# tobwei/APTAI

Measured on AMD Instinct MI355X. Metric: utterances/sec (10 s @ 16 kHz) train-step, higher is better.
Workload: dtype bf16

## Files before the change

### aptai_amd/csrc/gemm.hip

```cpp
#include <stdlib.h>

#include <mutex>
#include <set>

#include "common.h"
#include "gemm_common.h"

using namespace aptai_gemm;

namespace {

#ifdef APTAI_STAMPS
__device__ unsigned long long g_stamps[4096 * 8];
#define APTAI_STAMP(slot)                                                                          \
    do {                                                                                           \
        if (threadIdx.x == 0 && blockIdx.x < 4096 && blockIdx.y == 0 && blockIdx.z == 0)           \
            g_stamps[blockIdx.x * 8 + (slot)] = wall_clock64();                                    \
    } while (0)
extern "C" int aptai_debug_read_stamps(void* host_out) {
    return hipMemcpyFromSymbol(host_out, HIP_SYMBOL(g_stamps), sizeof(g_stamps)) == hipSuccess ? 0 : 1;
}
#else
#define APTAI_STAMP(slot) do {} while (0)
#endif

void epi_trace(const GemmArgs& g, int tile) {
    static const bool on = getenv("APTAI_EPI_TRACE") != nullptr;
    if (!on) return;
    static std::mutex mu;
    static std::set<int> seen;
    const int w = g.flags | (g.out_pre ? EPX_PRE : 0) | (g.colscale_n > 0 ? EPX_CS : 0);
    std::lock_guard<std::mutex> lk(mu);
    if (!seen.insert(w).second) return;
    bool listed = false;
#define APTAI_EPI_CASE(W) listed = listed || (w == (W));
    APTAI_EPI_WORDS(APTAI_EPI_CASE)
#undef APTAI_EPI_CASE
    fprintf(stderr, "[aptai epi] flag word 0x%x (tile %d, %d x %d x %d): %s\n", w, tile, g.M, g.N, g.K, listed ? "compiled" : "RUN-TIME form");
}

template <bool A_KM, bool B_KM, bool OUT_F32, int BM_T = 128>
__device__ __forceinline__ void gemm_tile_body(GemmArgs g, const int bid, const int batch, const int split) {
    extern __shared__ __attribute__((aligned(16))) char smem[];
    APTAI_STAMP(0);
    const int tid = threadIdx.x;
    const int lane = tid & 63;
    const int wave = __builtin_amdgcn_readfirstlane(tid >> 6);
    const int wm = wave >> 1, wn = wave & 1;

    int tile_m, tile_n;
    raster2d(bid, g.tiles_m, g.tiles_n, g.raster_gm, tile_m, tile_n);
    constexpr int NI = BM_T / 32;
    constexpr int WM = BM_T / 2;
    constexpr int NA_IT = BM_T / 32;
    constexpr int A_BYTES_T = BM_T * BK * 2;
    constexpr int STAGE_T = A_BYTES_T + BN * BK * 2;
    constexpr int NPASS = BM_T / 16;
    static_assert(BM_T == 128 || (BM_T == 64 && !A_KM), "64-row tiles are built for K-contiguous A only");
    constexpr bool RING5 = A_KM && B_KM && BM_T == 128 && APTAI_GEMM_RING5;
    const int m0 = tile_m * BM_T, n0 = tile_n * BN;

    if (batch >= 0) {
        const int bo = batch / g.nb_inner, bi = batch % g.nb_inner;
        g.A += bo * g.sA[0] + bi * g.sA[1];
        g.B += bo * g.sB[0] + bi * g.sB[1];
        const long co = bo * g.sC[0] + bi * g.sC[1];
        g.C = (OUT_F32 && !(g.flags & APTAI_EPI_SPLIT_OUT)) ? (void*)((float*)g.C + co) : (void*)((bf16_t*)g.C + co);
        if (g.out_pre) g.out_pre += co;
        if (g.bias) g.bias += bo * g.sBias[0] + bi * g.sBias[1];
        if (g.residual) g.residual += bo * g.sR[0] + bi * g.sR[1];
        if (g.aux) g.aux += bo * g.sAux[0] + bi * g.sAux[1];
    }
    const int total_kt = g.K / BK;
    const int kt_begin = split * g.ktiles_per_split;
    int kt_end = kt_begin + g.ktiles_per_split;
    kt_end = kt_end < total_kt ? kt_end : total_kt;
    const int nk = kt_end - kt_begin;

    f32x4 acc[NI][4];
#pragma unroll
    for (int i = 0; i < NI; ++i)
#pragma unroll
// ... 40 lines not shown
            }
#pragma unroll
            for (int it = 0; it < 2; ++it) {
                __builtin_amdgcn_global_load_lds(GLB_PTR(hb[it]), LDS_PTR(dst + HALF_T / 2 + it * (NTHREADS * 16)), 16, 0, 0);
                hb[it] += hstepB;
            }
        };
        uint32_t frag_off[16];
        {
            const int gq = lane >> 4, li = lane & 15, qq = li >> 2, pp = li & 3;
            const int k_lo = gq * 8 + qq, k_hi = k_lo + 4;
            const int sub = (pp & 1) << 3;
#pragma unroll
            for (int f = 0; f < 8; ++f) {
                const int is_b = f >> 2, idx = f & 3;
                const int row_base = is_b ? wn * 64 + idx * 16 : wm * WM + idx * 16;
                const int ch = (row_base >> 3) + (pp >> 1);
                frag_off[2 * f] = (uint32_t)(is_b * (HALF_T / 2) + k_lo * 256 + ((ch ^ km_swz(k_lo)) << 4) + sub);
                frag_off[2 * f + 1] = (uint32_t)(is_b * (HALF_T / 2) + k_hi * 256 + ((ch ^ km_swz(k_hi)) << 4) + sub);
            }
        }
        const uint32_t ring_base = (uint32_t)(uintptr_t)(__attribute__((address_space(3))) const char*)smem;
        const int nh = 2 * nk;
        if (nh > 0) { stage_half(0); stage_half(1); }
        if (nh > 2) stage_half(2);
        int s0 = 0;
        for (int kt = 0; kt < nk; ++kt) {
            if (kt + 1 < nk) asm volatile("s_waitcnt vmcnt(4) lgkmcnt(0)" ::: "memory");
            else asm volatile("s_waitcnt vmcnt(0) lgkmcnt(0)" ::: "memory");
            __builtin_amdgcn_s_barrier();
            asm volatile("" ::: "memory");
            const int s1 = s0 + 1 >= 5 ? s0 - 4 : s0 + 1, s2 = s0 + 2 >= 5 ? s0 - 3 : s0 + 2, s3 = s0 + 3 >= 5 ? s0 - 2 : s0 + 3,
                      s4 = s0 + 4 >= 5 ? s0 - 1 : s0 + 4;
            if (2 * kt + 3 < nh) stage_half(s3);
            if (2 * kt + 4 < nh) stage_half(s4);
            if (wave_active) {
                short4v fr[2][16];
#pragma unroll
                for (int hh = 0; hh < 2; ++hh) {
                    const uint32_t base = ring_base + (uint32_t)((hh ? s1 : s0) * HALF_T);
#pragma unroll
                    for (int f = 0; f < 16; ++f)
                        asm volatile("ds_read_b64_tr_b16 %0, %1" : "=v"(fr[hh][f]) : "v"(base + frag_off[f]));
                }
#define APTAI_TIE8(h, o) "+v"(fr[h][o]), "+v"(fr[h][o + 1]), "+v"(fr[h][o + 2]), "+v"(fr[h][o + 3]), "+v"(fr[h][o + 4]), \
                         "+v"(fr[h][o + 5]), "+v"(fr[h][o + 6]), "+v"(fr[h][o + 7])
#pragma unroll
                for (int hh = 0; hh < 2; ++hh) {
                    if (hh == 0) asm volatile("s_waitcnt lgkmcnt(15)" : APTAI_TIE8(0, 0), APTAI_TIE8(0, 8));
                    else asm volatile("s_waitcnt lgkmcnt(0)" : APTAI_TIE8(1, 0), APTAI_TIE8(1, 8));
                    bf16x8 af[NI], bfr[4];
#pragma unroll
                    for (int i = 0; i < NI; ++i) {
                        const short4v lo4 = fr[hh][2 * i], hi4 = fr[hh][2 * i + 1];
                        af[i] = __builtin_bit_cast(bf16x8, (short8v){lo4[0], lo4[1], lo4[2], lo4[3], hi4[0], hi4[1], hi4[2], hi4[3]});
                    }
#pragma unroll
                    for (int j = 0; j < 4; ++j) {
                        const short4v lo4 = fr[hh][8 + 2 * j], hi4 = fr[hh][8 + 2 * j + 1];
                        bfr[j] = __builtin_bit_cast(bf16x8, (short8v){lo4[0], lo4[1], lo4[2], lo4[3], hi4[0], hi4[1], hi4[2], hi4[3]});
                    }
#pragma unroll
                    for (int i = 0; i < NI; ++i)
#pragma unroll
                        for (int j = 0; j < 4; ++j)
                            acc[i][j] = __builtin_amdgcn_mfma_f32_16x16x32_bf16(bfr[j], af[i], acc[i][j], 0, 0, 0);
                }
#undef APTAI_TIE8
            }
            s0 = s2;
        }
        asm volatile("s_waitcnt vmcnt(0) lgkmcnt(0)" ::: "memory");
        __syncthreads();
    } else {
    if (nk > 0) stage(smem);
    for (int kt = 0; kt < nk; ++kt) {
        asm volatile("s_waitcnt vmcnt(0)" ::: "memory");
        __syncthreads();
        const int cur = kt & 1;
        if (kt + 1 < nk) stage(smem + (cur ^ 1) * STAGE_T);
        const char* sa = smem + cur * STAGE_T;
        const char* sb = sa + A_BYTES_T;
        if (wave_active) {
            if constexpr (!A_KM && !B_KM && APTAI_GEMM_HOIST) {
                bf16x8 af[2][NI], bfr[2][4];
#pragma unroll
                for (int ks = 0; ks < 2; ++ks) {
#pragma unroll
                    for (int j = 0; j < 4; ++j) bfr[ks][j] = read_frag<B_KM>(sb, wn * 64 + j * 16, ks, lane);
#pragma unroll
                    for (int i = 0; i < NI; ++i) af[ks][i] = read_frag<A_KM>(sa, wm * WM + i * 16, ks, lane);
                }
                __builtin_amdgcn_sched_barrier(0);
#pragma unroll
// ... 196 lines not shown
        }
        if (late) for (int i = 0; i < g.exp_sleep; ++i) __builtin_amdgcn_s_sleep(31);
    }
#endif
    gemm_tile_body<A_KM, B_KM, OUT_F32>(g, xcd_remap(blockIdx.x, g.tiles_m * g.tiles_n), gridDim.y > 1 ? (int)blockIdx.y : -1,
                                        blockIdx.z);
}

constexpr int SMEM_M64_BYTES = 2 * (64 + BN) * BK * 2;
template <bool B_KM, bool OUT_F32>
__global__ __launch_bounds__(NTHREADS, 3) void gemm_kernel_m64(GemmArgs g) {
    gemm_tile_body<false, B_KM, OUT_F32, 64>(g, xcd_remap(blockIdx.x, g.tiles_m * g.tiles_n), gridDim.y > 1 ? (int)blockIdx.y : -1,
                                             blockIdx.z);
}

constexpr int MAX_GROUP = 8;
struct GroupArgs {
    GemmArgs p[MAX_GROUP];
    int tile_end[MAX_GROUP];
    int n, total;
};

template <bool A_KM, bool B_KM, bool OUT_F32>
__global__ __launch_bounds__(NTHREADS, 3) void gemm_grouped_kernel(GroupArgs ga) {
    const int bid = xcd_remap(blockIdx.x, ga.total);
    int pi = 0;
#pragma unroll
    for (int i = 1; i < MAX_GROUP; ++i)
        if (i < ga.n && bid >= ga.tile_end[i - 1]) pi = i;
    const int first = pi ? ga.tile_end[pi - 1] : 0;
    gemm_tile_body<A_KM, B_KM, OUT_F32>(ga.p[pi], bid - first, -1, 0);
}

__global__ void splitk_reduce_kernel(const float* __restrict__ slabs, float* __restrict__ out, long n4, long slab_stride4,
                                     int nsplit, int accumulate) {
    const long stride = (long)gridDim.x * blockDim.x;
    for (long i = (long)blockIdx.x * blockDim.x + threadIdx.x; i < n4; i += stride) {
        f32x4 s = accumulate ? ((const f32x4*)out)[i] : (f32x4){0.f, 0.f, 0.f, 0.f};
        for (int k = 0; k < nsplit; ++k) s += ((const f32x4*)slabs)[(long)k * slab_stride4 + i];
        ((f32x4*)out)[i] = s;
    }
}

template <bool B_KM, bool OUT_F32>
int launch_gemm_m64(GemmArgs g, int nbatch, int nsplit, hipStream_t stream) {
    auto kern = gemm_kernel_m64<B_KM, OUT_F32>;
    g.tiles_m = (int)ceil_div(g.M, 64);
    dim3 grid(g.tiles_m * g.tiles_n, nbatch, nsplit);
    APTAI_LAUNCH(kern, grid, dim3(NTHREADS), SMEM_M64_BYTES, stream, g);
    APTAI_CHECK_LAUNCH("gemm_kernel_m64");
    return APTAI_OK;
}

template <bool A_KM, bool B_KM, bool OUT_F32>
// ... 890 lines not shown
                      "aptai_gemm_bf16: EPI_SPLIT_OUT needs out_f32, tile 128 / 192 / 256, 3 or 6 pieces and ldc >= pieces * N (bf16 elements)");
    APTAI_REQUIRE(d->colscale_n >= 0 && d->colscale_n % 8 == 0 && d->colscale_n <= d->N && (d->colscale_n == 0 || !d->out_f32),
                  "aptai_gemm_bf16: colscale_n must be a multiple of 8 within N, bf16 output only");
    memset(&g, 0, sizeof(g));
    g.A = (const bf16_t*)d->A; g.lda = d->lda;
    g.B = (const bf16_t*)d->B; g.ldb = d->ldb;
    g.C = d->C; g.ldc = d->ldc;
    g.M = (int)d->M; g.N = (int)d->N; g.K = (int)d->K;
    g.bias = d->bias;
    g.residual = (const bf16_t*)d->residual; g.ldr = d->ldr;
    g.out_pre = (bf16_t*)d->out_pre;
    g.aux = (const bf16_t*)d->aux; g.ldaux = d->ldaux;
    g.flags = d->flags;
    g.seed0 = (uint32_t)d->seed; g.seed1 = (uint32_t)(d->seed >> 32);
    g.salt = aptai_seed_salt(stream);
    g.thr16 = drop_thr16(d->dropout_p);
    g.dscale = drop_scale(g.thr16);
    if (g.thr16 == 0) g.flags &= ~APTAI_EPI_DROPOUT;
    g.alpha = d->alpha;
    g.colscale_n = d->colscale_n; g.colscale = d->colscale;
    g.split_pieces = d->split_out_pieces;
    g.split_bcol = (d->flags & APTAI_EPI_SPLIT_OUT) ? d->split_out_bcol : 0;
    g.hash_ld = d->N; g.hash_n0 = 0;
    g.tiles_m = (int)ceil_div(d->M, BM);
    g.tiles_n = (int)ceil_div(d->N, BN);
    {
        static int raster = -2;
        if (raster == -2) {
            const char* e = getenv("APTAI_GEMM_RASTER");
            raster = e ? atoi(e) : -1;
        }
        g.raster_gm = raster;
    }
    const int total_kt = g.K / BK;
    nsplit = d->split_k > 0 ? d->split_k : 1;
    if (nsplit > total_kt) nsplit = total_kt;
    g.ktiles_per_split = (int)ceil_div(total_kt, nsplit);
    nsplit = (int)ceil_div(total_kt, g.ktiles_per_split);

    nbatch = 1;
    g.nb_inner = 1;
    if (d->batch_outer > 1 || d->batch_inner > 1) {
        const int bo = d->batch_outer > 0 ? d->batch_outer : 1, bi = d->batch_inner > 0 ? d->batch_inner : 1;
        nbatch = bo * bi;
        g.nb_inner = bi;
        for (int l = 0; l < 2; ++l) {
// ... 33 lines not shown
                a.N = n1; a.tile = 256;
                b.N = rem; b.tile = 128;
                b.B = (const char*)d->B + (d->b_kmajor ? n1 * 2 : n1 * d->ldb * 2);
                b.C = (char*)d->C + n1 * 2;
                if (d->out_pre) b.out_pre = (char*)d->out_pre + n1 * 2;
                if (d->bias) b.bias = d->bias + n1;
                if (d->residual) b.residual = (const char*)d->residual + n1 * 2;
                if (d->aux) b.aux = (const char*)d->aux + n1 * 2;
                const int rc = gemm_bf16_one(&a, stream_, d->N, 0);
                if (rc != APTAI_OK) return rc;
                return gemm_bf16_one(&b, stream_, d->N, (int)n1);
            }
        }
    }
    return gemm_bf16_one(d, stream_, d ? d->N : 0, 0);
}

static int gemm_bf16_one(const aptai_gemm_desc* d, void* stream_, long hash_ld, int hash_n0) {
    hipStream_t stream = (hipStream_t)stream_;
    GemmArgs g;
    int nbatch = 1, nsplit = 1;
    const int brc = build_args(d, g, nbatch, nsplit, stream_);
    if (brc != APTAI_OK) return brc;
    g.hash_ld = hash_ld; g.hash_n0 = hash_n0;
    const bool f32 = d->out_f32 != 0;
    float* final_out = (float*)d->C;
    int tile = d->tile;
    if (tile == 0) {
        static int env_tile = -1;
        if (env_tile < 0) {
            const char* e = getenv("APTAI_GEMM_TILE");
            env_tile = e ? atoi(e) : 0;
        }
        tile = env_tile;
    }
    if (tile == 0) {
        const long t256 = ceil_div(d->M, T2_BM) * ceil_div(d->N, T2_BN) * nbatch * nsplit;
        const long t128 = ceil_div(d->M, BM) * ceil_div(d->N, BN) * nbatch * nsplit;
        const double e256 = (double)t256 / (double)(ceil_div(t256, 256) * 256);
        const double e128 = (double)t128 / (double)(ceil_div(t128, 512) * 512);
        static double f256 = -1.0;
        if (f256 < 0) {
            const char* e = getenv("APTAI_GEMM_F256");
            f256 = e ? atof(e) : 1.25;
        }
        tile = (d->M >= 256 && d->N >= 256 && f256 * e256 > e128) ? 256 : 128;
// ... 54 lines not shown
        else if (d->a_kmajor && d->b_kmajor) rc = f32 ? launch_gemm256<true, true, true>(g, nbatch, nsplit, stream) : launch_gemm256<true, true, false>(g, nbatch, nsplit, stream);
        else APTAI_FAIL(APTAI_ERR_INVALID, "aptai_gemm_bf16: A K-major with B K-contiguous is not built");
    } else
    if (!d->a_kmajor && !d->b_kmajor) rc = f32 ? launch_gemm<false, false, true>(g, nbatch, nsplit, stream) : launch_gemm<false, false, false>(g, nbatch, nsplit, stream);
    else if (!d->a_kmajor && d->b_kmajor) rc = f32 ? launch_gemm<false, true, true>(g, nbatch, nsplit, stream) : launch_gemm<false, true, false>(g, nbatch, nsplit, stream);
    else if (d->a_kmajor && d->b_kmajor) rc = f32 ? launch_gemm<true, true, true>(g, nbatch, nsplit, stream) : launch_gemm<true, true, false>(g, nbatch, nsplit, stream);
    else APTAI_FAIL(APTAI_ERR_INVALID, "aptai_gemm_bf16: A K-major with B K-contiguous is not built");
    if (rc != APTAI_OK) return rc;
    if (f32 && (nsplit > 1 || d->accumulate)) {
        const long n4 = (long)d->M * d->N / 4;
        int blocks = (int)(n4 / 256 < 2048 ? (n4 + 255) / 256 : 2048);
        APTAI_LAUNCH(splitk_reduce_kernel, dim3(blocks), dim3(256), 0, stream, (const float*)d->workspace, final_out,
                           n4, g.slab_stride / 4, nsplit, d->accumulate ? 1 : 0);
        APTAI_CHECK_LAUNCH("splitk_reduce_kernel");
    }
    return APTAI_OK;
}

extern "C" int aptai_gemm_bf16_grouped(const aptai_gemm_desc* descs, int n, void* stream_) {
    hipStream_t stream = (hipStream_t)stream_;
    APTAI_REQUIRE(descs != nullptr && n >= 1 && n <= MAX_GROUP, "aptai_gemm_bf16_grouped: need 1..%d problems, got %d", MAX_GROUP, n);
    GroupArgs ga;
    memset(&ga, 0, sizeof(ga));
    int total = 0;
    for (int i = 0; i < n; ++i) {
        const aptai_gemm_desc* d = descs + i;
        int nbatch = 1, nsplit = 1;
        const int brc = build_args(d, ga.p[i], nbatch, nsplit, stream_);
        if (brc != APTAI_OK) return brc;
        if (ga.p[i].raster_gm < 0) ga.p[i].raster_gm = (d->a_kmajor && d->b_kmajor) ? 8 : 0;
        APTAI_REQUIRE(nbatch == 1 && nsplit == 1 && !d->accumulate, "aptai_gemm_bf16_grouped: problem %d: no batching, split-K or accumulate", i);
        APTAI_REQUIRE(d->a_kmajor == descs[0].a_kmajor && d->b_kmajor == descs[0].b_kmajor && (d->out_f32 != 0) == (descs[0].out_f32 != 0),
                      "aptai_gemm_bf16_grouped: problem %d: all problems must share the operand layout and output type", i);
        total += ga.p[i].tiles_m * ga.p[i].tiles_n;
        ga.tile_end[i] = total;
    }
    ga.n = n;
    ga.total = total;
    const bool f32 = descs[0].out_f32 != 0, akm = descs[0].a_kmajor != 0, bkm = descs[0].b_kmajor != 0;
    APTAI_REQUIRE(!(akm && !bkm), "aptai_gemm_bf16_grouped: A K-major with B K-contiguous is not built");
#define APTAI_GROUPED(AK, BK_, F)                                                                                      \
    do {                                                                                                              \
        auto kern = gemm_grouped_kernel<AK, BK_, F>;                                                                  \
        constexpr int smem = smem_for<AK, BK_>();                                                                     \
        static bool attr_set = false;                                                                                 \
        if (!attr_set) {                                                                                              \
            (void)hipFuncSetAttribute((const void*)kern, hipFuncAttributeMaxDynamicSharedMemorySize, smem);                  \
            attr_set = true;                                                                                          \
        }                                                                                                             \
        APTAI_LAUNCH(kern, dim3(total), dim3(NTHREADS), smem, stream, ga);                                            \
    } while (0)
    if (!akm && !bkm) { if (f32) APTAI_GROUPED(false, false, true); else APTAI_GROUPED(false, false, false); }
    else if (!akm && bkm) { if (f32) APTAI_GROUPED(false, true, true); else APTAI_GROUPED(false, true, false); }
    else { if (f32) APTAI_GROUPED(true, true, true); else APTAI_GROUPED(true, true, false); }
#undef APTAI_GROUPED
    APTAI_CHECK_LAUNCH("gemm_grouped_kernel");
    return APTAI_OK;
}

extern "C" int64_t aptai_gemm_sk_workspace_bytes(void) { return sk_workspace_bytes(); }

extern "C" int aptai_gemm_sk_status(void* sk_workspace, void* stream, int* status_out) {
    APTAI_REQUIRE(sk_workspace != nullptr && status_out != nullptr, "aptai_gemm_sk_status: null pointer");
// ... 14 lines not shown
```

### aptai_amd/csrc/gemm_common.h

```cpp
#pragma once
#include "common.h"

namespace aptai_gemm {


#ifndef APTAI_GEMM_HOIST
#define APTAI_GEMM_HOIST 1
#endif
constexpr int BM = 128, BN = 128, BK = 64;
constexpr int NTHREADS = 256;
constexpr int STAGE_BYTES = (BM * BK + BN * BK) * 2;
constexpr int OPER_BYTES = BM * BK * 2;
constexpr int EPI_PITCH = BN * 4 + 16;
constexpr int SMEM_BYTES = BM * EPI_PITCH > 2 * STAGE_BYTES ? BM * EPI_PITCH : 2 * STAGE_BYTES;
#ifndef APTAI_GEMM_RING5
#define APTAI_GEMM_RING5 1
#endif
#ifndef APTAI_GEMM_M64_ASM
#define APTAI_GEMM_M64_ASM 1
#endif
#ifndef APTAI_GEMM192_ASM
#define APTAI_GEMM192_ASM 1
#endif
constexpr int RING_HALF_BYTES = (BM + BN) * 32 * 2;
// ... 3 lines not shown

struct GemmArgs {
    const bf16_t* A; long lda;
    const bf16_t* B; long ldb;
    void* C; long ldc;
    int M, N, K;
    const float* bias;
    const bf16_t* residual; long ldr;
    bf16_t* out_pre;
    const bf16_t* aux; long ldaux;
    int flags;
    uint32_t seed0, seed1, thr16;
    const uint32_t* salt;
    float dscale;
    float alpha;
    int ktiles_per_split;
    long slab_stride;
    int tiles_m, tiles_n;
    int raster_gm;
    long hash_ld; int hash_n0;
    int colscale_n; float colscale;
    int split_pieces;
    int split_bcol;
#ifdef APTAI_EXP_STAGGER
    int exp_sleep;
    unsigned* exp_cu_count;
#endif
    int nb_inner;
    long sA[2], sB[2], sC[2], sBias[2], sR[2], sAux[2];
};



__device__ __forceinline__ int km_swz(int krow) { return ((krow & 3) << 2) | ((krow >> 2) & 3); }

__device__ __forceinline__ void gelu_fast_both(float x, float& y, float& dy) {
    const float xc = __builtin_amdgcn_fmed3f(x, -7.0f, 7.0f);
    const float x2 = xc * xc;
    const float s = gelu_sig(xc, x2);
    float q = fmaf(5.0f * APTAI_GELU_A5, x2, 3.0f * APTAI_GELU_A3);
    q = fmaf(q, x2, APTAI_GELU_A1);
    y = x * s;
    dy = fmaf(fmaf(-s, s, s), xc * q, s);
}

constexpr int EPX_PRE = 1 << 16;
// ... 208 lines not shown
```

### aptai_amd/ops.py

```python
from __future__ import annotations

import ctypes
from typing import Optional

import torch

from . import _lib

EPI_BIAS, EPI_GELU, EPI_RESIDUAL, EPI_DROPOUT, EPI_DGELU, EPI_ALPHA, EPI_PRE_DGELU, EPI_MUL_AUX, EPI_RESIDUAL_F32, EPI_SPLIT_OUT, EPI_BIAS_ROW = 1, 2, 4, 8, 16, 32, 64, 128, 256, 512, 1024

c_void_p, c_i64, c_int, c_float, c_u64 = (ctypes.c_void_p, ctypes.c_int64, ctypes.c_int, ctypes.c_float,
                                          ctypes.c_uint64)


class GemmDesc(ctypes.Structure):
    _fields_ = [("A", c_void_p), ("lda", c_i64), ("B", c_void_p), ("ldb", c_i64), ("C", c_void_p), ("ldc", c_i64),
                ("M", c_i64), ("N", c_i64), ("K", c_i64),
                ("a_kmajor", c_int), ("b_kmajor", c_int), ("out_f32", c_int), ("flags", c_int),
                ("bias", c_void_p), ("residual", c_void_p), ("ldr", c_i64), ("out_pre", c_void_p),
                ("aux", c_void_p), ("ldaux", c_i64), ("alpha", c_float), ("dropout_p", c_float), ("seed", c_u64),
                ("split_k", c_int), ("accumulate", c_int), ("workspace", c_void_p), ("workspace_bytes", c_i64),
                ("batch_outer", c_int), ("batch_inner", c_int),
                ("batch_stride_a", c_i64 * 2), ("batch_stride_b", c_i64 * 2), ("batch_stride_c", c_i64 * 2),
                ("batch_stride_bias", c_i64 * 2), ("batch_stride_res", c_i64 * 2), ("batch_stride_aux", c_i64 * 2),
                ("tile", c_int), ("colscale_n", c_int), ("colscale", c_float),
                ("sk_workspace", c_void_p), ("sk_workspace_bytes", c_i64), ("split_out_pieces", c_int), ("split_out_bcol", c_int)]


TILE_STREAMK = 257
_SK_WS = {}


def _sk_workspace(device) -> torch.Tensor:
    key = (str(device), _stream())
    ws = _SK_WS.get(key)
    if ws is None:
        ws = torch.zeros(int(_lib.lib().aptai_gemm_sk_workspace_bytes()), device=device, dtype=torch.uint8)
        _SK_WS[key] = ws
    return ws


def gemm_sk_check(device=None) -> None:
    for (d, st), ws in list(_SK_WS.items()):
        if device is not None and d != str(device):
            continue
        out = ctypes.c_int(0)
        _lib.check(_lib.lib().aptai_gemm_sk_status(c_void_p(ws.data_ptr()), c_void_p(st), ctypes.byref(out)), "aptai_gemm_sk_status")
        if out.value != 0:
            raise _lib.AptaiHipError("aptai_gemm_bf16 (stream-K): a wait for another workgroup's partial tile timed out; "
# ... 135 lines not shown
        return False


def gemm(a: torch.Tensor, b: torch.Tensor, M: int, N: int, K: int, **kw) -> torch.Tensor:
    d = GemmDesc()
    out, _ws_keep = _gemm_desc(d, a, b, M, N, K, **kw)
    pr = _probe
    if pr is not None and pr.key == (bool(d.a_kmajor), bool(d.b_kmajor), bool(d.out_f32)) and not torch.cuda.is_current_stream_capturing():
        e0, e1 = torch.cuda.Event(enable_timing=True), torch.cuda.Event(enable_timing=True)
        e0.record()
        _lib.check(_lib.lib().aptai_gemm_bf16(ctypes.byref(d), c_void_p(_stream())), "aptai_gemm_bf16")
        e1.record()
        batch = kw.get("batch")
        nb = (batch.get("outer", 1) * batch.get("inner", 1)) if batch else 1
        pr.records.append((2.0 * M * N * K * nb, e0, e1))
        return out
    _lib.check(_lib.lib().aptai_gemm_bf16(ctypes.byref(d), c_void_p(_stream())), "aptai_gemm_bf16")
    return out


def gemm_grouped(problems) -> list:
    problems = list(problems)
    descs = (GemmDesc * len(problems))()
    outs, keep = [], []
    flops = 0.0
    for d, (a, b, M, N, K, kw) in zip(descs, problems):
        out, ws = _gemm_desc(d, a, b, M, N, K, **kw)
        outs.append(out)
        keep.append(ws)
        flops += 2.0 * M * N * K
    pr = _probe
    d0 = descs[0]
    if pr is not None and pr.key == (bool(d0.a_kmajor), bool(d0.b_kmajor), bool(d0.out_f32)) and not torch.cuda.is_current_stream_capturing():
        e0, e1 = torch.cuda.Event(enable_timing=True), torch.cuda.Event(enable_timing=True)
        e0.record()
        _lib.check(_lib.lib().aptai_gemm_bf16_grouped(descs, len(problems), c_void_p(_stream())), "aptai_gemm_bf16_grouped")
        e1.record()
        pr.records.append((flops, e0, e1))
        return outs
    _lib.check(_lib.lib().aptai_gemm_bf16_grouped(descs, len(problems), c_void_p(_stream())), "aptai_gemm_bf16_grouped")
    return outs


_ONES = {}


def ones_kmajor(K: int, device) -> torch.Tensor:
    key = (K, str(device))
    t = _ONES.get(key)
    if t is None:
        t = torch.ones((K, 8), device=device, dtype=torch.bfloat16)
        _ONES[key] = t
    return t
# ... 727 lines not shown
```

### aptai_amd/wav2vec2.py

```python
from __future__ import annotations

import json
import math
import os
from types import SimpleNamespace
from typing import List, Optional, Tuple

import numpy as np
import torch
import torch.nn as nn

from . import hostlogic, ops
from .config import W2V2Config


def _round_up(x: int, m: int) -> int:
    return (x + m - 1) // m * m


def _rows_with_zero_slack(rows: int, C: int, dev, slack: int = 8) -> torch.Tensor:
    t = torch.empty((rows, C), device=dev, dtype=torch.bfloat16)
    t[rows - slack:].zero_()
    return t

# ... 234 lines not shown
        dctx = ops.gemm(d_att_out, w.wo, M, H, H, b_kmajor=True)
        st = self.attn_state
        dqkv = ops.attention_bwd(s.qkv, self.lens, s.ctx, dctx, s.lse, g.B, g.Tp, H, heads, q_prescaled=True, dropout_p=p_att,
                                 seed=_seed(self.seed, 1), dctx_zero_beyond_len=st is None or not st.seen)
        if dprobs is not None:
            ops.attention_probs_bwd(s.qkv, self.lens, s.lse[0], dprobs.contiguous(), g.B, g.Tp, H, heads, q_prescaled=True,
                                    dropout_p=p_att, seed=_seed(self.seed, 1), dqkv=dqkv)
            if st is not None:
                st.seen = True
        attn_in = s.n1 if pre else s.x
        if not grouped:
            dwqkv, dbqkv = on_side(lambda: (ops.gemm(dqkv, attn_in, 3 * H, H, M, a_kmajor=True, b_kmajor=True, out_f32=True, split_k=sk[0]),
                                            ops.colsum(dqkv, M, 3 * H)))
        if pre:
            dn1 = ops.gemm(dqkv, w.wqkv, M, H, 3 * H, b_kmajor=True)
            dx, _, dg1, db1 = ops.layernorm_bwd(dn1, s.x, s.m1, s.r1, ln1w, dres=ds1)
        else:
            dx = ops.gemm(dqkv, w.wqkv, M, H, 3 * H, b_kmajor=True, residual=ds1)
        if grouped and defer_wgrad:
            pending = SimpleNamespace(d_ffn_out=d_ffn_out, hact=s.hact, du=du, ffn_in=ffn_in, d_att_out=d_att_out, ctx=s.ctx, dqkv=dqkv,
                                      attn_in=attn_in, M=M, H=H, I=I)
            return dx, (dg1, db1, dg2, db2), pending
        if grouped:
            tn = dict(a_kmajor=True, b_kmajor=True, out_f32=True)
            ones = ops.ones_kmajor(M, dy.device)
            dw2, dw1, dwo, dwqkv, r2, r1, ro, rq = ops.gemm_grouped([
                (d_ffn_out, s.hact, H, I, M, tn), (du, ffn_in, I, H, M, tn), (d_att_out, s.ctx, H, H, M, tn),
                (dqkv, attn_in, 3 * H, H, M, tn),
                (ones, d_ffn_out, 8, H, M, tn), (ones, du, 8, I, M, tn), (ones, d_att_out, 8, H, M, tn),
                (ones, dqkv, 8, 3 * H, M, tn)])
            dbias2, dbias1, dbo, dbqkv = r2[0], r1[0], ro[0], rq[0]
        main.wait_stream(side)
        return dx, (dg1, db1, dg2, db2, dwqkv[0:H], dwqkv[H:2 * H], dwqkv[2 * H:3 * H], dbqkv[0:H], dbqkv[H:2 * H],
                    dbqkv[2 * H:3 * H], dwo, dbo, dw1, dbias1, dw2, dbias2)


    @staticmethod
    def bwd_wgrad(p):
        M, H, I = p.M, p.H, p.I
        tn = dict(a_kmajor=True, b_kmajor=True, out_f32=True)
        ones = ops.ones_kmajor(M, p.du.device)
        dw2, dw1, dwo, dwqkv, r2, r1, ro, rq = ops.gemm_grouped([
            (p.d_ffn_out, p.hact, H, I, M, tn), (p.du, p.ffn_in, I, H, M, tn), (p.d_att_out, p.ctx, H, H, M, tn),
            (p.dqkv, p.attn_in, 3 * H, H, M, tn),
            (ones, p.d_ffn_out, 8, H, M, tn), (ones, p.du, 8, I, M, tn), (ones, p.d_att_out, 8, H, M, tn),
            (ones, p.dqkv, 8, 3 * H, M, tn)])
        dbias2, dbias1, dbo, dbqkv = r2[0], r1[0], ro[0], rq[0]
        return (dwqkv[0:H], dwqkv[H:2 * H], dwqkv[2 * H:3 * H], dbqkv[0:H], dbqkv[H:2 * H], dbqkv[2 * H:3 * H], dwo, dbo, dw1, dbias1,
                dw2, dbias2)


_SIDE_STREAMS = {}
_GROUPED_WGRAD = os.environ.get("APTAI_GROUPED_WGRAD", "1") != "0"
_PRE_DGELU = os.environ.get("APTAI_PRE_DGELU", "1") != "0"
_SPEC_ON_DEVICE = os.environ.get("APTAI_SPEC_ON_DEVICE", "1") != "0"
_USE_SIDE_STREAM = os.environ.get("APTAI_SIDE_STREAM", "0") != "0"


def _side_stream(device):
    st = _SIDE_STREAMS.get(device)
    if st is None:
        st = torch.cuda.Stream(device=device)
        _SIDE_STREAMS[device] = st
    return st


class _FrontImpl:

    def __init__(self, cfg, geom, lens_i32, spec, training, seed, model):
        self.cfg, self.g, self.lens, self.spec, self.training, self.seed, self.model = cfg, geom, lens_i32, spec, training, seed, model
# ... 732 lines not shown
```

### include/aptai_hip.h

```cpp
#ifndef APTAI_HIP_H
#define APTAI_HIP_H
#include <stdint.h>

#ifdef __cplusplus
extern "C" {
#endif

typedef enum {
    APTAI_OK = 0,
    APTAI_ERR_INVALID = -1,
    APTAI_ERR_LAUNCH = -2,
    APTAI_ERR_NO_DEVICE = -3
} aptai_status;

const char* aptai_last_error(void);
int aptai_version(void);
int aptai_device_check(char* name, int name_len);
int aptai_set_seed_salt(void* stream, const void* device_ptr_2xu32);
int aptai_set_frame_bounds(void* stream, const void* device_ptr_2xi32);

enum {
    APTAI_EPI_BIAS = 1,
    APTAI_EPI_GELU = 2,
    APTAI_EPI_RESIDUAL = 4,
// ... 12 lines not shown
    const void* B; int64_t ldb;
    void* C; int64_t ldc;
    int64_t M, N, K;
    int a_kmajor, b_kmajor, out_f32;
    int flags;
    const float* bias;
    const void* residual; int64_t ldr;
    void* out_pre;
    const void* aux; int64_t ldaux;
    float alpha;
    float dropout_p; uint64_t seed;
    int split_k;
    int accumulate;
    void* workspace; int64_t workspace_bytes;
    int batch_outer, batch_inner;
    int64_t batch_stride_a[2], batch_stride_b[2], batch_stride_c[2], batch_stride_bias[2], batch_stride_res[2],
        batch_stride_aux[2];
    int tile;
    int colscale_n; float colscale;
    void* sk_workspace;
    int64_t sk_workspace_bytes;
    int split_out_pieces;
    int split_out_bcol;
} aptai_gemm_desc;

int aptai_gemm_bf16(const aptai_gemm_desc* desc, void* stream);
int aptai_gemm_bf16_grouped(const aptai_gemm_desc* descs, int n, void* stream);
int64_t aptai_gemm_workspace_bytes(int64_t M, int64_t N, int split_k);
int64_t aptai_gemm_sk_workspace_bytes(void);
int aptai_gemm_sk_status(void* sk_workspace, void* stream, int* status_out);

int aptai_split_f32(const float* x, int64_t ldx, int64_t rows, int64_t cols, int pattern, int pieces, int act, void* out, int64_t ldo,
                    void* stream);
int aptai_bias_act_res_f32(const float* x, int64_t ldx, const float* bias, const float* res, int64_t ldr, float* y, int64_t ldy,
                           int64_t rows, int64_t cols, int act, const int32_t* lens, int64_t rows_per_b, void* stream);
int aptai_softmax_rows_f32(float* s, const int32_t* lens, int64_t B, int64_t heads, int64_t Tp, void* stream);
int aptai_softmax_split_f32(const float* s, const int32_t* lens, int64_t B, int64_t heads, int64_t Tp, int pieces, void* out, int64_t ldo,
                            void* stream);
int aptai_attention_exact_fwd(const void* qkv_split, int64_t ld, const int32_t* lens, void* ctx_split, int64_t ldo, int64_t B, int64_t Tp,
                              int64_t H, int64_t heads, int pieces, float scale, void* stream);
int aptai_conv0_fwd_f32(const float* audio, int64_t B, int64_t S, const float* weight, const float* bias, const float* gamma,
                        const float* beta, int mode, float eps, float* out, int64_t T_real, int64_t T_alloc, const float* stats,
                        void* stream);
int aptai_conv0_fwd_split(const float* audio, int64_t B, int64_t S, const float* weight, const float* bias, const float* gamma,
                          const float* beta, int mode, float eps, void* out_split, int pieces, int64_t T_real, int64_t T_alloc,
                          const float* stats, void* stream);
// ... 154 lines not shown
```

Before: 1734.

## Fuse bias-gradient column sums into the grouped wgrad GEMM and add wide-tile wgrad kernel

Bias gradients were previously computed as four extra grouped GEMM problems that multiply a ones matrix against each activation gradient. Now the K-major ring loop feeds the A fragments into extra MFMAs against a ones vector, only on tiles with tile_n==0 and wn==0, and writes per-row sums to a colsum buffer. This removes the four extra problems and their second read of the activation gradients, at the cost of extra MFMAs and registers in those tiles. The launch bound of the grouped kernel drops from 3 to 2 blocks per CU for the K-major ring path, and a separate 256-wide, 512-thread wgrad kernel is added behind an env flag that is off by default.

```diff
diff --git a/aptai_amd/csrc/gemm.hip b/aptai_amd/csrc/gemm.hip
--- a/aptai_amd/csrc/gemm.hip
+++ b/aptai_amd/csrc/gemm.hip
@@ -39,7 +39,21 @@
     fprintf(stderr, "[aptai epi] flag word 0x%x (tile %d, %d x %d x %d): %s\n", w, tile, g.M, g.N, g.K, listed ? "compiled" : "RUN-TIME form");
 }
 
-template <bool A_KM, bool B_KM, bool OUT_F32, int BM_T = 128>
+__device__ __forceinline__ void colsum_step(const bf16x8 (&af)[4], f32x4 (&cs)[4]) {
+    const bf16x8 ones = __builtin_bit_cast(bf16x8, (short8v){0x3f80, 0x3f80, 0x3f80, 0x3f80, 0x3f80, 0x3f80, 0x3f80, 0x3f80});
+#pragma unroll
+    for (int i = 0; i < 4; ++i) cs[i] = __builtin_amdgcn_mfma_f32_16x16x32_bf16(af[i], ones, cs[i], 0, 0, 0);
+}
+__device__ __forceinline__ void colsum_store(float* __restrict__ colsum, const f32x4 (&cs)[4], const int mbase, const int M, const int lane) {
+    if ((lane & 15) != 0) return;
+#pragma unroll
+    for (int i = 0; i < 4; ++i) {
+        const int m = mbase + i * 16 + (lane >> 4) * 4;
+        if (m < M) *(f32x4*)(colsum + m) = cs[i];
+    }
+}
+
+template <bool A_KM, bool B_KM, bool OUT_F32, int BM_T = 128, bool CSUM = false>
 __device__ __forceinline__ void gemm_tile_body(GemmArgs g, const int bid, const int batch, const int split) {
     extern __shared__ __attribute__((aligned(16))) char smem[];
     APTAI_STAMP(0);
@@ -58,6 +72,7 @@
     constexpr int NPASS = BM_T / 16;
     static_assert(BM_T == 128 || (BM_T == 64 && !A_KM), "64-row tiles are built for K-contiguous A only");
     constexpr bool RING5 = A_KM && B_KM && BM_T == 128 && APTAI_GEMM_RING5;
+    static_assert(!CSUM || RING5, "column sums are built into the K-major / K-major ring loop only");
     const int m0 = tile_m * BM_T, n0 = tile_n * BN;
 
     if (batch >= 0) {
@@ -144,6 +159,10 @@
         }
         const uint32_t ring_base = (uint32_t)(uintptr_t)(__attribute__((address_space(3))) const char*)smem;
         const int nh = 2 * nk;
+        const bool do_cs = CSUM && g.colsum != nullptr && tile_n == 0 && wn == 0 && m0 + wm * WM < g.M;
+        f32x4 cs[4];
+#pragma unroll
+        for (int i = 0; i < 4; ++i) cs[i] = (f32x4){0.f, 0.f, 0.f, 0.f};
         if (nh > 0) { stage_half(0); stage_half(1); }
         if (nh > 2) stage_half(2);
         int s0 = 0;
@@ -187,11 +206,15 @@
 #pragma unroll
                         for (int j = 0; j < 4; ++j)
                             acc[i][j] = __builtin_amdgcn_mfma_f32_16x16x32_bf16(bfr[j], af[i], acc[i][j], 0, 0, 0);
+                    if constexpr (CSUM)
+                        if (do_cs) colsum_step(af, cs);
                 }
 #undef APTAI_TIE8
             }
             s0 = s2;
         }
+        if constexpr (CSUM)
+            if (do_cs) colsum_store(g.colsum, cs, m0 + wm * WM, g.M, lane);
         asm volatile("s_waitcnt vmcnt(0) lgkmcnt(0)" ::: "memory");
         __syncthreads();
     } else {
@@ -434,14 +457,198 @@
 };
 
 template <bool A_KM, bool B_KM, bool OUT_F32>
-__global__ __launch_bounds__(NTHREADS, 3) void gemm_grouped_kernel(GroupArgs ga) {
+__global__ __launch_bounds__(NTHREADS, (A_KM && B_KM && APTAI_GEMM_RING5) ? 2 : 3) void gemm_grouped_kernel(GroupArgs ga) {
     const int bid = xcd_remap(blockIdx.x, ga.total);
     int pi = 0;
 #pragma unroll
     for (int i = 1; i < MAX_GROUP; ++i)
         if (i < ga.n && bid >= ga.tile_end[i - 1]) pi = i;
     const int first = pi ? ga.tile_end[pi - 1] : 0;
-    gemm_tile_body<A_KM, B_KM, OUT_F32>(ga.p[pi], bid - first, -1, 0);
+    gemm_tile_body<A_KM, B_KM, OUT_F32, 128, A_KM && B_KM && OUT_F32 && APTAI_GEMM_RING5>(ga.p[pi], bid - first, -1, 0);
+}
+
+#ifndef APTAI_WGRAD_RING
+#define APTAI_WGRAD_RING 6
+#endif
+#ifndef APTAI_WGRAD_WIDE_DEFAULT
+#define APTAI_WGRAD_WIDE_DEFAULT 0
+#endif
+constexpr int W_THREADS = 512;
+constexpr int W_BN = 256;
+constexpr int W_PART = 32 * 128 * 2;
+constexpr int W_HALF = 3 * W_PART;
+constexpr int W_SLOTS = APTAI_WGRAD_RING;
+constexpr int W_SMEM = W_SLOTS * W_HALF;
+constexpr int W_EPI_PITCH = W_BN * 4 + 16;
+static_assert(W_SLOTS == 5 || W_SLOTS == 6, "the counted waits are written for a ring of 5 or 6 half-stages");
+static_assert(64 * W_EPI_PITCH <= W_SMEM, "half of the fp32 epilogue tile (64 rows) must fit the ring");
+
+__device__ __forceinline__ void wgrad_wide_tile_body(const GemmArgs& g, const int bid) {
+    extern __shared__ __attribute__((aligned(16))) char smem[];
+    const int tid = threadIdx.x;
+    const int lane = tid & 63;
+    const int wave = __builtin_amdgcn_readfirstlane(tid >> 6);
+    const int wm = wave >> 2, wn = wave & 3;
+    int tile_m, tile_n;
+    raster2d(bid, g.tiles_m, g.tiles_n, g.raster_gm, tile_m, tile_n);
+    const int m0 = tile_m * BM, n0 = tile_n * W_BN;
+    const int nk = g.K / BK;
+
+    f32x4 acc[4][4], cs[4];
+#pragma unroll
+    for (int i = 0; i < 4; ++i) {
+        cs[i] = (f32x4){0.f, 0.f, 0.f, 0.f};
+#pragma unroll
+        for (int j = 0; j < 4; ++j) acc[i][j] = (f32x4){0.f, 0.f, 0.f, 0.f};
+    }
+    const bool wave_active = (m0 + wm * 64 < g.M) && (n0 + wn * 64 < g.N);
+    const bool do_cs = g.colsum != nullptr && tile_n == 0 && wn == 0 && m0 + wm * 64 < g.M;
+
+    const bf16_t *ha, *hb0, *hb1;
+    {
+        const int krow = tid >> 4, sw = ((tid & 15) ^ km_swz(krow)) << 3;
+        auto src = [&](const bf16_t* base, long ld, int row0, int rows_total) {
+            int col = row0 + sw;
+            col = col <= rows_total - 8 ? col : rows_total - 8;
+            return base + (long)krow * ld + col;
+        };
+        ha = src(g.A, g.lda, m0, g.M);
+        hb0 = src(g.B, g.ldb, n0, g.N);
+        hb1 = src(g.B, g.ldb, n0 + 128, g.N);
+    }
+    const long hstepA = 32 * (long)g.lda, hstepB = 32 * (long)g.ldb;
+    const int wave_base_tid = wave * 64;
+    auto stage_half = [&](int slot) {
+        char* dst = smem + slot * W_HALF + wave_base_tid * 16;
+        __builtin_amdgcn_global_load_lds(GLB_PTR(ha), LDS_PTR(dst), 16, 0, 0);
+        __builtin_amdgcn_global_load_lds(GLB_PTR(hb0), LDS_PTR(dst + W_PART), 16, 0, 0);
+        __builtin_amdgcn_global_load_lds(GLB_PTR(hb1), LDS_PTR(dst + 2 * W_PART), 16, 0, 0);
+        ha += hstepA;
+        hb0 += hstepB;
+        hb1 += hstepB;
+    };
+    uint32_t frag_off[16];
+    {
+        const int gq = lane >> 4, li = lane & 15, qq = li >> 2, pp = li & 3;
+        const int k_lo = gq * 8 + qq, k_hi = k_lo + 4;
+        const int sub = (pp & 1) << 3;
+#pragma unroll
+        for (int f = 0; f < 8; ++f) {
+            const int is_b = f >> 2, idx = f & 3;
+            const int row_base = is_b ? (wn & 1) * 64 + idx * 16 : wm * 64 + idx * 16;
+            const int part = is_b ? (1 + (wn >> 1)) * W_PART : 0;
+            const int ch = (row_base >> 3) + (pp >> 1);
+            frag_off[2 * f] = (uint32_t)(part + k_lo * 256 + ((ch ^ km_swz(k_lo)) << 4) + sub);
+            frag_off[2 * f + 1] = (uint32_t)(part + k_hi * 256 + ((ch ^ km_swz(k_hi)) << 4) + sub);
+        }
+    }
+    const uint32_t ring_base = (uint32_t)(uintptr_t)(__attribute__((address_space(3))) const char*)smem;
+    const int nh = 2 * nk;
+    auto wrap = [](int s) { return s >= W_SLOTS ? s - W_SLOTS : s; };
+#pragma unroll
+    for (int h = 0; h < W_SLOTS - 1; ++h)
+        if (h < nh) stage_half(h);
+    short4v fa[16], fb[16];
+    auto read_half = [&](short4v (&fr)[16], const int slot) __attribute__((always_inline)) {
+        const uint32_t base = ring_base + (uint32_t)(slot * W_HALF);
+#pragma unroll
+        for (int f = 0; f < 16; ++f) asm volatile("ds_read_b64_tr_b16 %0, %1" : "=v"(fr[f]) : "v"(base + frag_off[f]));
+    };
+    auto mfma_half = [&](const short4v (&fr)[16]) __attribute__((always_inline)) {
+        bf16x8 af[4], bfr[4];
+#pragma unroll
+        for (int i = 0; i < 4; ++i) {
+            af[i] = combine_tr(fr[2 * i], fr[2 * i + 1]);
+            bfr[i] = combine_tr(fr[8 + 2 * i], fr[8 + 2 * i + 1]);
+        }
+#pragma unroll
+        for (int i = 0; i < 4; ++i)
+#pragma unroll
+            for (int j = 0; j < 4; ++j)
+                acc[i][j] = __builtin_amdgcn_mfma_f32_16x16x32_bf16(bfr[j], af[i], acc[i][j], 0, 0, 0);
+        if (do_cs) colsum_step(af, cs);
+    };
+#define APTAI_TIE16(fr) "+v"(fr[0]), "+v"(fr[1]), "+v"(fr[2]), "+v"(fr[3]), "+v"(fr[4]), "+v"(fr[5]), "+v"(fr[6]), "+v"(fr[7]), "+v"(fr[8]), \
+                        "+v"(fr[9]), "+v"(fr[10]), "+v"(fr[11]), "+v"(fr[12]), "+v"(fr[13]), "+v"(fr[14]), "+v"(fr[15])
+    if (W_SLOTS - 1 <= nh) {
+        if constexpr (W_SLOTS == 6) asm volatile("s_waitcnt vmcnt(12)" ::: "memory");
+        else asm volatile("s_waitcnt vmcnt(9)" ::: "memory");
+    } else {
+        asm volatile("s_waitcnt vmcnt(0)" ::: "memory");
+    }
+    __builtin_amdgcn_s_barrier();
+    asm volatile("" ::: "memory");
+    if (wave_active) read_half(fa, 0);
+    int s0 = 0;
+    for (int j = 0; j < nk; ++j) {
+        if (2 * j + W_SLOTS - 2 < nh) {
+            if constexpr (W_SLOTS == 6) asm volatile("s_waitcnt vmcnt(6) lgkmcnt(0)" ::: "memory");
+            else asm volatile("s_waitcnt vmcnt(3) lgkmcnt(0)" ::: "memory");
+        } else {
+            asm volatile("s_waitcnt vmcnt(0) lgkmcnt(0)" ::: "memory");
+        }
+        if (wave_active) asm volatile("" : APTAI_TIE16(fa));
+        __builtin_amdgcn_s_barrier();
+        asm volatile("" ::: "memory");
+        if (2 * j + W_SLOTS - 1 < nh) stage_half(wrap(s0 + W_SLOTS - 1));
+        if (2 * j + W_SLOTS < nh) stage_half(s0);
+        if (wave_active) {
+            read_half(fb, wrap(s0 + 1));
+            __builtin_amdgcn_sched_barrier(0);
+            mfma_half(fa);
+            __builtin_amdgcn_sched_barrier(0);
+            asm volatile("s_waitcnt lgkmcnt(0)" : APTAI_TIE16(fb) : : "memory");
+            if (j + 1 < nk) read_half(fa, wrap(s0 + 2));
+            __builtin_amdgcn_sched_barrier(0);
+            mfma_half(fb);
+        }
+        s0 = wrap(s0 + 2);
+    }
+#undef APTAI_TIE16
+    if (do_cs) colsum_store(g.colsum, cs, m0 + wm * 64, g.M, lane);
+    asm volatile("s_waitcnt vmcnt(0) lgkmcnt(0)" ::: "memory");
+    __syncthreads();
+
+    const int cl = (tid & 31) * 8;
+    const int n = n0 + cl;
+#pragma unroll
+    for (int p = 0; p < 2; ++p) {
+        if (p) __syncthreads();
+        if (wm == p) {
+#pragma unroll
+            for (int i = 0; i < 4; ++i) {
+                const int ml = i * 16 + (lane & 15);
+#pragma unroll
+                for (int j = 0; j < 4; ++j) {
+                    const int nl = wn * 64 + j * 16 + (lane >> 4) * 4;
+                    *(f32x4*)(smem + ml * W_EPI_PITCH + nl * 4) = acc[i][j];
+                }
+            }
+        }
+        __syncthreads();
+#pragma unroll
+        for (int step = 0; step < 4; ++step) {
+            const int ml = step * 16 + (tid >> 5);
+            const int m = m0 + p * 64 + ml;
+            if (m < g.M && n < g.N) {
+                const f32x4 v0 = *(const f32x4*)(smem + ml * W_EPI_PITCH + cl * 4);
+                const f32x4 v1 = *(const f32x4*)(smem + ml * W_EPI_PITCH + cl * 4 + 16);
+                float* C = (float*)g.C + (long)m * g.ldc + n;
+                *(f32x4*)C = v0;
+                *(f32x4*)(C + 4) = v1;
+            }
+        }
+    }
+}
+
+__global__ __launch_bounds__(W_THREADS, 1) void wgrad_wide_grouped_kernel(GroupArgs ga) {
+    const int bid = xcd_remap(blockIdx.x, ga.total);
+    int pi = 0;
+#pragma unroll
+    for (int i = 1; i < MAX_GROUP; ++i)
+        if (i < ga.n && bid >= ga.tile_end[i - 1]) pi = i;
+    const int first = pi ? ga.tile_end[pi - 1] : 0;
+    wgrad_wide_tile_body(ga.p[pi], bid - first);
 }
 
 __global__ void splitk_reduce_kernel(const float* __restrict__ slabs, float* __restrict__ out, long n4, long slab_stride4,
@@ -1378,6 +1585,10 @@
     g.split_pieces = d->split_out_pieces;
     g.split_bcol = (d->flags & APTAI_EPI_SPLIT_OUT) ? d->split_out_bcol : 0;
     g.hash_ld = d->N; g.hash_n0 = 0;
+    if (d->colsum)
+        APTAI_REQUIRE(d->a_kmajor && d->b_kmajor && d->out_f32 && (uintptr_t)d->colsum % 16 == 0,
+                      "aptai_gemm_bf16: colsum needs K-major A and B, fp32 output and a 16-B aligned pointer");
+    g.colsum = d->colsum;
     g.tiles_m = (int)ceil_div(d->M, BM);
     g.tiles_n = (int)ceil_div(d->N, BN);
     {
@@ -1457,6 +1668,7 @@
     int nbatch = 1, nsplit = 1;
     const int brc = build_args(d, g, nbatch, nsplit, stream_);
     if (brc != APTAI_OK) return brc;
+    APTAI_REQUIRE(d->colsum == nullptr, "aptai_gemm_bf16: colsum is produced by the grouped launch only (aptai_gemm_bf16_grouped)");
     g.hash_ld = hash_ld; g.hash_n0 = hash_n0;
     const bool f32 = d->out_f32 != 0;
     float* final_out = (float*)d->C;
@@ -1557,6 +1769,9 @@
     APTAI_REQUIRE(descs != nullptr && n >= 1 && n <= MAX_GROUP, "aptai_gemm_bf16_grouped: need 1..%d problems, got %d", MAX_GROUP, n);
     GroupArgs ga;
     memset(&ga, 0, sizeof(ga));
+    static const bool wide_on = getenv("APTAI_WGRAD_TILE") ? atoi(getenv("APTAI_WGRAD_TILE")) == 256 : APTAI_WGRAD_WIDE_DEFAULT != 0;
+    bool wide = wide_on && descs[0].a_kmajor && descs[0].b_kmajor && descs[0].out_f32;
+    for (int i = 0; i < n && wide; ++i) wide = descs[i].flags == 0;
     int total = 0;
     for (int i = 0; i < n; ++i) {
         const aptai_gemm_desc* d = descs + i;
@@ -1567,6 +1782,7 @@
         APTAI_REQUIRE(nbatch == 1 && nsplit == 1 && !d->accumulate, "aptai_gemm_bf16_grouped: problem %d: no batching, split-K or accumulate", i);
         APTAI_REQUIRE(d->a_kmajor == descs[0].a_kmajor && d->b_kmajor == descs[0].b_kmajor && (d->out_f32 != 0) == (descs[0].out_f32 != 0),
                       "aptai_gemm_bf16_grouped: problem %d: all problems must share the operand layout and output type", i);
+        if (wide) ga.p[i].tiles_n = (int)ceil_div(d->N, W_BN);
         total += ga.p[i].tiles_m * ga.p[i].tiles_n;
         ga.tile_end[i] = total;
     }
@@ -1574,6 +1790,17 @@
     ga.total = total;
     const bool f32 = descs[0].out_f32 != 0, akm = descs[0].a_kmajor != 0, bkm = descs[0].b_kmajor != 0;
     APTAI_REQUIRE(!(akm && !bkm), "aptai_gemm_bf16_grouped: A K-major with B K-contiguous is not built");
+    if (wide) {
+        auto kern = wgrad_wide_grouped_kernel;
+        static bool attr_set = false;
+        if (!attr_set) {
+            (void)hipFuncSetAttribute((const void*)kern, hipFuncAttributeMaxDynamicSharedMemorySize, W_SMEM);
+            attr_set = true;
+        }
+        APTAI_LAUNCH(kern, dim3(total), dim3(W_THREADS), W_SMEM, stream, ga);
+        APTAI_CHECK_LAUNCH("wgrad_wide_grouped_kernel");
+        return APTAI_OK;
+    }
 #define APTAI_GROUPED(AK, BK_, F)                                                                                      \
     do {                                                                                                              \
         auto kern = gemm_grouped_kernel<AK, BK_, F>;                                                                  \
diff --git a/aptai_amd/csrc/gemm_common.h b/aptai_amd/csrc/gemm_common.h
--- a/aptai_amd/csrc/gemm_common.h
+++ b/aptai_amd/csrc/gemm_common.h
@@ -49,6 +49,7 @@
     int colscale_n; float colscale;
     int split_pieces;
     int split_bcol;
+    float* colsum;
 #ifdef APTAI_EXP_STAGGER
     int exp_sleep;
     unsigned* exp_cu_count;
diff --git a/aptai_amd/ops.py b/aptai_amd/ops.py
--- a/aptai_amd/ops.py
+++ b/aptai_amd/ops.py
@@ -24,7 +24,8 @@
                 ("batch_stride_a", c_i64 * 2), ("batch_stride_b", c_i64 * 2), ("batch_stride_c", c_i64 * 2),
                 ("batch_stride_bias", c_i64 * 2), ("batch_stride_res", c_i64 * 2), ("batch_stride_aux", c_i64 * 2),
                 ("tile", c_int), ("colscale_n", c_int), ("colscale", c_float),
-                ("sk_workspace", c_void_p), ("sk_workspace_bytes", c_i64), ("split_out_pieces", c_int), ("split_out_bcol", c_int)]
+                ("sk_workspace", c_void_p), ("sk_workspace_bytes", c_i64), ("split_out_pieces", c_int), ("split_out_bcol", c_int),
+                ("colsum", c_void_p)]
 
 
 TILE_STREAMK = 257
@@ -206,13 +207,19 @@
 def gemm_grouped(problems) -> list:
     problems = list(problems)
     descs = (GemmDesc * len(problems))()
-    outs, keep = [], []
+    outs, keep, sums = [], [], []
     flops = 0.0
     for d, (a, b, M, N, K, kw) in zip(descs, problems):
+        if kw.get("colsum"):
+            kw = {k: v for k, v in kw.items() if k != "colsum"}
+            cs = torch.empty(M, device=a.device, dtype=torch.float32)
+            d.colsum = cs.data_ptr()
+            sums.append(cs)
         out, ws = _gemm_desc(d, a, b, M, N, K, **kw)
         outs.append(out)
         keep.append(ws)
         flops += 2.0 * M * N * K
+    outs += sums
     pr = _probe
     d0 = descs[0]
     if pr is not None and pr.key == (bool(d0.a_kmajor), bool(d0.b_kmajor), bool(d0.out_f32)) and not torch.cuda.is_current_stream_capturing():
diff --git a/aptai_amd/wav2vec2.py b/aptai_amd/wav2vec2.py
--- a/aptai_amd/wav2vec2.py
+++ b/aptai_amd/wav2vec2.py
@@ -280,14 +280,10 @@
                                       attn_in=attn_in, M=M, H=H, I=I)
             return dx, (dg1, db1, dg2, db2), pending
         if grouped:
-            tn = dict(a_kmajor=True, b_kmajor=True, out_f32=True)
-            ones = ops.ones_kmajor(M, dy.device)
-            dw2, dw1, dwo, dwqkv, r2, r1, ro, rq = ops.gemm_grouped([
+            tn = dict(a_kmajor=True, b_kmajor=True, out_f32=True, colsum=True)
+            dw2, dw1, dwo, dwqkv, dbias2, dbias1, dbo, dbqkv = ops.gemm_grouped([
                 (d_ffn_out, s.hact, H, I, M, tn), (du, ffn_in, I, H, M, tn), (d_att_out, s.ctx, H, H, M, tn),
-                (dqkv, attn_in, 3 * H, H, M, tn),
-                (ones, d_ffn_out, 8, H, M, tn), (ones, du, 8, I, M, tn), (ones, d_att_out, 8, H, M, tn),
-                (ones, dqkv, 8, 3 * H, M, tn)])
-            dbias2, dbias1, dbo, dbqkv = r2[0], r1[0], ro[0], rq[0]
+                (dqkv, attn_in, 3 * H, H, M, tn)])
         main.wait_stream(side)
         return dx, (dg1, db1, dg2, db2, dwqkv[0:H], dwqkv[H:2 * H], dwqkv[2 * H:3 * H], dbqkv[0:H], dbqkv[H:2 * H],
                     dbqkv[2 * H:3 * H], dwo, dbo, dw1, dbias1, dw2, dbias2)
@@ -296,14 +292,10 @@
     @staticmethod
     def bwd_wgrad(p):
         M, H, I = p.M, p.H, p.I
-        tn = dict(a_kmajor=True, b_kmajor=True, out_f32=True)
-        ones = ops.ones_kmajor(M, p.du.device)
-        dw2, dw1, dwo, dwqkv, r2, r1, ro, rq = ops.gemm_grouped([
+        tn = dict(a_kmajor=True, b_kmajor=True, out_f32=True, colsum=True)
+        dw2, dw1, dwo, dwqkv, dbias2, dbias1, dbo, dbqkv = ops.gemm_grouped([
             (p.d_ffn_out, p.hact, H, I, M, tn), (p.du, p.ffn_in, I, H, M, tn), (p.d_att_out, p.ctx, H, H, M, tn),
-            (p.dqkv, p.attn_in, 3 * H, H, M, tn),
-            (ones, p.d_ffn_out, 8, H, M, tn), (ones, p.du, 8, I, M, tn), (ones, p.d_att_out, 8, H, M, tn),
-            (ones, p.dqkv, 8, 3 * H, M, tn)])
-        dbias2, dbias1, dbo, dbqkv = r2[0], r1[0], ro[0], rq[0]
+            (p.dqkv, p.attn_in, 3 * H, H, M, tn)])
         return (dwqkv[0:H], dwqkv[H:2 * H], dwqkv[2 * H:3 * H], dbqkv[0:H], dbqkv[H:2 * H], dbqkv[2 * H:3 * H], dwo, dbo, dw1, dbias1,
                 dw2, dbias2)
 
diff --git a/include/aptai_hip.h b/include/aptai_hip.h
--- a/include/aptai_hip.h
+++ b/include/aptai_hip.h
@@ -58,6 +58,7 @@
     int64_t sk_workspace_bytes;
     int split_out_pieces;
     int split_out_bcol;
+    float* colsum;
 } aptai_gemm_desc;
 
 int aptai_gemm_bf16(const aptai_gemm_desc* desc, void* stream);
```

Result: no change. 1751 (median of 6 runs) (+1.0%).
